# RioWong/PointCloudProcess

Measured on AMD Instinct MI355X. Metric: Mcorrespondences/s + ICP iter/s, 50M-vs-50M fp32 @ 1/2/4/8 MI355X, higher is better.
Workload: dtype f32

## Files before the change

include/pcp.h:

```cpp
#ifndef PCP_H
#define PCP_H

#include <stddef.h>
#include <stdint.h>

#ifdef __cplusplus
extern "C" {
#endif

#define PCP_ABI_VERSION 1

enum pcp_status {
    PCP_OK = 0,
    PCP_ERR_ARG = -1,
    PCP_ERR_HIP = -2,
    PCP_ERR_NOMEM = -3,
    PCP_ERR_EMPTY = -4,
    PCP_ERR_UNSUPPORTED = -5,
    PCP_ERR_ICP = -6,
    PCP_ERR_CAPACITY = -7
};

#define PCP_AOS48_STRIDE 48

// ... 139 lines not shown
                             int64_t nq, const uint64_t* keys_dev, const uint8_t* owner_dev, int rank,
                             int64_t lo, int64_t hi, const float* shard_xyz_dev, size_t shard_stride_bytes,
                             double* acc_dev);
int pcp_slab_guard(pcp_ctx* ctx, const double* T_dev, const double box_host[6], double lo,
                   double hi, int* flag_dev);
int pcp_icp_solve(const double acc_host[24], int do_scale, double dT_host[16]);
int pcp_icp_run(pcp_ctx* ctx, pcp_icp* icp, double T_inout[16], float rmax, int iters,
                int do_scale, double eps, float* err);
int pcp_icp_last_kernel_ms(const pcp_icp* icp, double* ms, int* launches);
int pcp_icp_step_dev(pcp_ctx* ctx, pcp_icp* icp, const double* T_dev, float rmax, double* acc_dev);
int pcp_icp_solve_dev(pcp_ctx* ctx, const double* acc_dev, int do_scale, double* T_dev, double* stats_dev);
int pcp_icp_run_dev(pcp_ctx* ctx, pcp_icp* icp, double* T_dev, float rmax, int iters, int do_scale,
                    double* stats_dev);
int pcp_icp_kernel_ms(pcp_ctx* ctx, pcp_icp* icp, double* ms, int* launches);
int pcp_icp_last_fallback(const pcp_icp* icp, int64_t* n);
int pcp_icp_last_searched(const pcp_icp* icp, int64_t* n);

int pcp_get_rot_icp(pcp_ctx* ctx, const void* src_aos48_dev, int64_t ns, int src_is_dense,
                    const void* temp_aos48_dev, int64_t nt, int temp_is_dense,
                    double mat_rot_host[16], float rmax, int iters, int do_scale,
                    double cell_size, float* err);

int pcp_pose_interpolate(double* rots_host, int64_t n, int64_t start, int64_t end);
int pcp_pose_lum_elch(double* rots_host, int64_t n, int64_t start, int64_t end, const double loop_host[16]);
int pcp_pose_loop_closure(double* ori_host, const uint64_t* ori_stamps_host, int64_t n_ori, const double* opt_host,
                          const uint64_t* opt_stamps_host, int64_t n_opt, int64_t window);

typedef struct pcp_grid pcp_grid;
int pcp_grid_create(pcp_ctx* ctx, pcp_grid** out);
int pcp_grid_destroy(pcp_grid* grid);
// ... 22 lines not shown
```

pointcloudprocess_amd/_lib.py:

```python
import ctypes as C
import os

HERE = os.path.dirname(os.path.abspath(__file__))
_AB = os.environ.get("PCP_AB") == "1" and bool(os.environ.get("PCP_LIB"))
LIB_PATH = os.environ["PCP_LIB"] if _AB else os.path.join(HERE, "libpcp.so")

PCP_OK = 0
_STATUS = {
    -1: "PCP_ERR_ARG", -2: "PCP_ERR_HIP", -3: "PCP_ERR_NOMEM", -4: "PCP_ERR_EMPTY",
    -5: "PCP_ERR_UNSUPPORTED", -6: "PCP_ERR_ICP", -7: "PCP_ERR_CAPACITY",
}

_vp, _i32, _i64, _sz, _f32, _f64, _u32 = (C.c_void_p, C.c_int, C.c_int64, C.c_size_t,
                                          C.c_float, C.c_double, C.c_uint32)
_P = C.POINTER
SIGNATURES = [
    ("pcp_abi_version", _i32, []),
    ("pcp_ctx_create", _i32, [_i32, _vp, _P(_vp)]),
    ("pcp_ctx_destroy", _i32, [_vp]),
    ("pcp_ctx_set_stream", _i32, [_vp, _vp]),
    ("pcp_ctx_stream", _vp, [_vp]),
    ("pcp_last_error", C.c_char_p, [_vp]),
    ("pcp_sync", _i32, [_vp]),
    ("pcp_malloc", _i32, [_vp, _P(_vp), _sz]),
# ... 57 lines not shown
    ("pcp_icp_keys", _i32, [_vp, _vp, _P(_f64), _f32, _i64, _vp]),
    ("pcp_icp_accumulate_keys", _i32, [_vp, _vp, _P(_f64), _vp, _i64, _i64, _vp, _sz, _vp]),
    ("pcp_icp_keys_dev", _i32, [_vp, _vp, _vp, _f32, _i64, _vp]),
    ("pcp_keys_owner", _i32, [_vp, _vp, _i64, _vp, _i32, _vp]),
    ("pcp_icp_accumulate_owned", _i32, [_vp, _vp, _vp, _sz, _i64, _vp, _vp, _i32, _i64, _i64, _vp, _sz, _vp]),
    ("pcp_slab_guard", _i32, [_vp, _vp, _P(_f64), _f64, _f64, _vp]),
    ("pcp_icp_solve", _i32, [_P(_f64), _i32, _P(_f64)]),
    ("pcp_icp_run", _i32, [_vp, _vp, _P(_f64), _f32, _i32, _i32, _f64, _P(_f32)]),
    ("pcp_icp_last_kernel_ms", _i32, [_vp, _P(_f64), _P(_i32)]),
    ("pcp_icp_step_dev", _i32, [_vp, _vp, _vp, _f32, _vp]),
    ("pcp_icp_solve_dev", _i32, [_vp, _vp, _i32, _vp, _vp]),
    ("pcp_icp_run_dev", _i32, [_vp, _vp, _vp, _f32, _i32, _i32, _vp]),
    ("pcp_icp_kernel_ms", _i32, [_vp, _vp, _P(_f64), _P(_i32)]),
    ("pcp_icp_last_fallback", _i32, [_vp, _P(_i64)]),
    ("pcp_icp_last_searched", _i32, [_vp, _P(_i64)]),
    ("pcp_fault_report_install", _i32, []),
    ("pcp_build_id", C.c_char_p, []),
    ("pcp_get_rot_icp", _i32, [_vp, _vp, _i64, _i32, _vp, _i64, _i32, _P(_f64), _f32, _i32, _i32,
                               _f64, _P(_f32)]),
]

_lib = None


class PcpError(RuntimeError):
    def __init__(self, code, msg):
        super().__init__(f"{_STATUS.get(code, code)}: {msg}")
        self.code = code


# ... 40 lines not shown
```

pointcloudprocess_amd/csrc/grid.hip:

```cpp
#include <cmath>
#include <vector>

#include <rocprim/device/device_radix_sort.hpp>
#include "sortcfg.hpp"

#include "grid.hpp"

namespace pcp {
namespace {

constexpr int kB = 256;

template <typename T>
__device__ __forceinline__ const T* pt_ptr(const T* base, size_t stride_bytes, int64_t i) {
    return (const T*)((const char*)base + (size_t)i * stride_bytes);
}

template <typename T>
__global__ void k_valid(const T* xyz, size_t stride, int64_t n_in, const int32_t* indices,
                        uint32_t* flag) {
    for (int64_t i = blockIdx.x * (int64_t)blockDim.x + threadIdx.x; i < n_in;
         i += (int64_t)gridDim.x * blockDim.x) {
        int64_t ci = indices ? indices[i] : i;
        const T* p = pt_ptr(xyz, stride, ci);
// ... 144 lines not shown
        bool on = (bits[i >> 5] >> (i & 31)) & 1u;
        brick[i] = on ? brick[i] : -1;
    }
}

constexpr int kChunk = 4096;
#ifndef PCP_SCAN_BLOCKS
#define PCP_SCAN_BLOCKS 16384
#endif
#ifndef PCP_BBOX_BLOCKS
#define PCP_BBOX_BLOCKS 4096
#endif
constexpr int64_t kScanBlocks = PCP_SCAN_BLOCKS;
constexpr int64_t kBboxBlocks = PCP_BBOX_BLOCKS;

__global__ void k_chunk_lo(const uint32_t* key, int64_t n, int64_t nchunk, uint32_t* lo) {
    for (int64_t p = blockIdx.x * (int64_t)blockDim.x + threadIdx.x; p <= n; p += (int64_t)gridDim.x * blockDim.x) {
        const int64_t kc = p < n ? (int64_t)key[p] : nchunk * kChunk;
        const int64_t kp = p > 0 ? (int64_t)key[p - 1] : -1;
        if (kc == kp) continue;
        const int64_t b0 = kp < 0 ? 0 : kp / kChunk + 1;
        const int64_t b1 = min(kc / kChunk, nchunk);
        for (int64_t b = b0; b <= b1; b++) lo[b] = (uint32_t)p;
    }
}

__global__ void __launch_bounds__(256) k_cell_starts(const uint32_t* __restrict__ key, const uint32_t* __restrict__ lo,
                                                     int64_t ncells1, uint32_t* __restrict__ cstart) {
    constexpr int kPer = kChunk / 256;
    __shared__ uint32_t s[kChunk];
    __shared__ uint32_t s_wmin[4];
    const int64_t c0 = (int64_t)blockIdx.x * kChunk;
// ... 38 lines not shown
        const int64_t c = c0 + e;
        if (c + 3 < ncells1) {
            *(uint4*)&cstart[c] = o;
        } else {
            if (c < ncells1) cstart[c] = o.x;
            if (c + 1 < ncells1) cstart[c + 1] = o.y;
            if (c + 2 < ncells1) cstart[c + 2] = o.z;
        }
    }
}

__global__ void k_far_sentinel(float4* pts, int64_t n) {
    pts[n] = make_float4(INFINITY, INFINITY, INFINITY, __int_as_float(0x7fffffff));
}

__global__ void k_cell_keys_rec(GridDesc g, const float* cxyz, size_t stride_f, const int32_t* mapping, int64_t n,
                                uint32_t* key, float4* rec, int32_t* mark) {
    for (int64_t i = blockIdx.x * (int64_t)blockDim.x + threadIdx.x; i < n;
         i += (int64_t)gridDim.x * blockDim.x) {
        const float* p = cxyz + stride_f * i;
        int cx, cy, cz;
        cell_of_point<float>(g, p, cx, cy, cz);
        key[i] = (uint32_t)cell_id(g, cx, cy, cz);
        rec[i] = make_float4(p[0], p[1], p[2], __int_as_float(mapping ? mapping[i] : (int32_t)i));
        if (mark) mark[brick_of(g, cx, cy, cz)] = 1;
    }
}


template <typename T>
__global__ void k_cell_keys(GridDesc g, const T* cxyz, size_t stride_t, int64_t n, uint32_t* key, uint32_t* val,
                            int32_t* mark) {
    for (int64_t i = blockIdx.x * (int64_t)blockDim.x + threadIdx.x; i < n;
         i += (int64_t)gridDim.x * blockDim.x) {
        int cx, cy, cz;
        cell_of_point<T>(g, cxyz + stride_t * i, cx, cy, cz);
        key[i] = (uint32_t)cell_id(g, cx, cy, cz);
        val[i] = (uint32_t)i;
        if (mark) mark[brick_of(g, cx, cy, cz)] = 1;
    }
}

// ... 169 lines not shown
    const int64_t dense_cap = std::min<int64_t>(((int64_t)1 << 31) - 2, std::max<int64_t>((int64_t)1 << 26, 16 * n));
    double ext[3];
    for (int a = 0; a < 3; a++) ext[a] = std::max(mx[a] - mn[a], 1e-9);
    const bool auto_h = !(cell_size > 0);
    double h = cell_size;
    if (auto_h) {
        const double target = 4.0;
        h = std::cbrt(ext[0] * ext[1] * ext[2] * target / std::max<double>((double)n, 1.0));
        double emax = std::max(ext[0], std::max(ext[1], ext[2]));
        if (!(h > emax * 1e-7)) h = emax * 1e-7;
        if (!(h > 0)) h = 1.0;
    }
    uint32_t* count = nullptr;
    uint32_t* rank = nullptr;
    uint32_t* skey = nullptr;
    if ((is_f64 && (rc = dmalloc(ctx, &rank, n + 1))) || (rc = dmalloc(ctx, &skey, n + 1))) {
        dfree(ctx, rank);
        dfree(ctx, cxyz);
        return fail(rc);
    }
    if ((rc = dmalloc(ctx, (typename Real<T>::V4**)&ix->pts, n + 1))) {
        dfree(ctx, rank); dfree(ctx, skey); dfree(ctx, cxyz);
        return fail(rc);
    }
    bool hooked = false;
    for (int attempt = 0; attempt < 3; attempt++) {
        GridDesc g{};
        while (!make_geometry(g, mn, mx, h, cap)) h *= 2.0;
        dfree(ctx, ix->brick); ix->brick = nullptr;
        dfree(ctx, count); count = nullptr;
        const int64_t ncells_dense = (int64_t)g.n[0] * g.n[1] * g.n[2];
// ... 46 lines not shown
            if (occ > 12.0) { h *= std::sqrt(4.0 / occ); redo = true; }
            else if (occ < 1.5) { h *= std::cbrt(4.0 / occ); redo = true; }
            if (redo) continue;
        }
        if (on_geom && *on_geom && !hooked) {
            hooked = true;
            if ((rc = (*on_geom)(g))) break;
        }
        if ((rc = dmalloc(ctx, &count, ncells + 2))) break;
        uint32_t* key1 = nullptr;
        uint32_t* val1 = nullptr;
        using V4 = typename Real<T>::V4;
        if (n > 0) {
            if ((rc = dmalloc(ctx, &key1, n))) break;
            if (is_f64 && (rc = dmalloc(ctx, &val1, n))) { dfree(ctx, key1); break; }
            float4* rec0 = nullptr;
            if (!is_f64 && (rc = dmalloc(ctx, &rec0, n))) { dfree(ctx, key1); break; }
            unsigned bits = 1;
            while (bits < 32 && ((uint64_t)1 << bits) <= (uint64_t)ncells) bits++;
            size_t tmp_bytes = 0;
            void* tmp = nullptr;
            if (is_f64) {
                hipLaunchKernelGGL(k_cell_keys<T>, dim3(grid_for(n, kB)), dim3(kB), 0, st, g, direct ? xyz : cxyz,
                                   direct ? stride / sizeof(T) : (size_t)3, n, skey, rank, g.dense ? ix->brick : nullptr);
                PCP_HIP(ctx, rocprim::radix_sort_pairs(nullptr, tmp_bytes, skey, key1, rank, val1, (size_t)n, 0u,
                                                       bits, st));
                if (!(rc = dmalloc(ctx, (char**)&tmp, tmp_bytes)))
                    PCP_HIP(ctx, rocprim::radix_sort_pairs(tmp, tmp_bytes, skey, key1, rank, val1, (size_t)n, 0u,
                                                           bits, st));
            } else {
                if (direct)
                    hipLaunchKernelGGL(k_cell_keys_rec, dim3(grid_for(n, kB)), dim3(kB), 0, st, g, (const float*)xyz,
                                       stride / sizeof(float), (const int32_t*)nullptr, n, skey, rec0, nullptr);
                else
                    hipLaunchKernelGGL(k_cell_keys_rec, dim3(grid_for(n, kB)), dim3(kB), 0, st, g, (const float*)cxyz,
                                       (size_t)3, (const int32_t*)ix->mapping, n, skey, rec0, nullptr);
                PCP_HIP(ctx, rocprim::radix_sort_pairs<RecSortConfig>(nullptr, tmp_bytes, skey, key1, rec0, (float4*)ix->pts,
                                                       (size_t)n, 0u, bits, st));
                if (!(rc = dmalloc(ctx, (char**)&tmp, tmp_bytes)))
                    PCP_HIP(ctx, rocprim::radix_sort_pairs<RecSortConfig>(tmp, tmp_bytes, skey, key1, rec0, (float4*)ix->pts,
                                                           (size_t)n, 0u, bits, st));
            }
            dfree(ctx, tmp);
            dfree(ctx, rec0);
            if (rc) { dfree(ctx, key1); dfree(ctx, val1); break; }
            if (!is_f64)
                hipLaunchKernelGGL(k_far_sentinel, dim3(1), dim3(1), 0, st, (float4*)ix->pts, n);
        }
        if (g.dense && is_f64)
            hipLaunchKernelGGL(k_brick_flag, dim3(grid_for(g.nbricks, kB)), dim3(kB), 0, st, ix->brick, g.nbricks);
        const int64_t nchunk = (ncells + 1 + kChunk - 1) / kChunk;
        uint32_t* lo = nullptr;
        if ((rc = dmalloc(ctx, &lo, nchunk + 1))) {
            dfree(ctx, key1); dfree(ctx, val1);
            break;
        }
        hipLaunchKernelGGL(k_chunk_lo, dim3(grid_for(n + 1, kB, kScanBlocks)), dim3(kB), 0, st, (const uint32_t*)key1, n,
                           nchunk, lo);
        hipLaunchKernelGGL(k_cell_starts, dim3((unsigned)nchunk), dim3(kB), 0, st, (const uint32_t*)key1,
                           (const uint32_t*)lo, ncells + 1, count);
        dfree(ctx, lo);
        g.cstart = count;
        if (g.dense && is_f64 && n > 0)
            hipLaunchKernelGGL(k_brick_rows, dim3(grid_for(g.nbricks, kB)), dim3(kB), 0, st, g, ix->brick);
        ix->g = g;
        ix->cstart = count;
        count = nullptr;
        if (is_f64) {
            if ((rc = dmalloc(ctx, &ix->sorted_j, n + 1))) { dfree(ctx, key1); dfree(ctx, val1); break; }
            if (n > 0)
                hipLaunchKernelGGL(k_gather<T>, dim3(grid_for(n, kB)), dim3(kB), 0, st, direct ? xyz : cxyz,
                                   direct ? stride / sizeof(T) : (size_t)3, (const uint32_t*)val1,
                                   (const int32_t*)ix->mapping, n, (V4*)ix->pts, ix->sorted_j, is_f64);
// ... 72 lines not shown
```

pointcloudprocess_amd/csrc/icp.hip:

```cpp
#include <cmath>
#include <cstdlib>
#include <cstring>
#include <vector>

#include <rocprim/device/device_radix_sort.hpp>
#include <rocprim/device/device_select.hpp>
#include <rocprim/iterator/counting_iterator.hpp>
#include "sortcfg.hpp"

#include "grid.hpp"
#include "wave_acc.hpp"

namespace pcp {
struct QXyz {
    float x, y, z;
};
}

struct pcp_icp {
    pcp_ctx* ctx = nullptr;
    pcp_ctx* owner = nullptr;
    const pcp_index* target = nullptr;
    int64_t nq = 0;
    int64_t nq_in = 0;
    pcp::QXyz* q = nullptr;
    int32_t* qidx = nullptr;
    uint32_t* cand = nullptr;
    bool narrow = false;
    float* pose_hist = nullptr;
    int64_t launches = 0;
    bool last_verified = false;
    int32_t* sv = nullptr;
    uint32_t* sv_count = nullptr;
    uint32_t* sv_off = nullptr;
    int32_t* svc = nullptr;
    int64_t sv_seg = 0;
    int64_t nseg_v = 0;
    int nb_ver = 0;
    int32_t* fb = nullptr;
    uint32_t* fb_count = nullptr;
    uint32_t* fb_off = nullptr;
// ... 1383 lines not shown
    if (!(mn >= lo && mx <= hi)) *flag = 1;
}

#ifndef PCP_QKEY_LOCAL
#define PCP_QKEY_LOCAL 1
#endif
#ifndef PCP_QBRICK
#define PCP_QBRICK 8
#endif
__host__ __device__ inline int64_t qbricks(const GridDesc& g, int a) { return (g.n[a] + PCP_QBRICK - 1) / PCP_QBRICK; }
__host__ __device__ inline uint32_t query_key_end(const GridDesc& g) {
    if (PCP_QBRICK != 4)
        return (uint32_t)(qbricks(g, 0) * qbricks(g, 1) * qbricks(g, 2) * PCP_QBRICK * PCP_QBRICK * PCP_QBRICK);
    return (uint32_t)(PCP_QKEY_LOCAL ? g.nbricks * 64 : g.nbricks);
}
__global__ void k_query_keys(GridDesc g, const float* q, size_t stride_f, int64_t n, uint32_t* key, float4* rec) {
    for (int64_t i = blockIdx.x * (int64_t)blockDim.x + threadIdx.x; i < n; i += (int64_t)gridDim.x * blockDim.x) {
        const float* p = q + (size_t)i * stride_f;
        const float x = p[0], y = p[1], z = p[2];
        const bool fin = isfinite(x) && isfinite(y) && isfinite(z);
        uint32_t k = query_key_end(g);
        if (fin) {
            const int cx = clampi((int)floorf(cell_f<float>(g, x, 0) - 0.5f), 0, g.n[0] - 1);
            const int cy = clampi((int)floorf(cell_f<float>(g, y, 1) - 0.5f), 0, g.n[1] - 1);
            const int cz = clampi((int)floorf(cell_f<float>(g, z, 2) - 0.5f), 0, g.n[2] - 1);
            if (PCP_QBRICK != 4) {
                constexpr int B = PCP_QBRICK;
                const int64_t b = ((int64_t)(cz / B) * qbricks(g, 1) + cy / B) * qbricks(g, 0) + cx / B;
                k = (uint32_t)(b * B * B * B + ((cz % B) * B + cy % B) * B + cx % B);
            } else {
                k = PCP_QKEY_LOCAL ? (uint32_t)(brick_of(g, cx, cy, cz) * 64 + local_of(cx, cy, cz))
                                   : (uint32_t)brick_of(g, cx, cy, cz);
            }
        }
        key[i] = k;
        rec[i] = make_float4(x, y, z, __int_as_float((int)i));
    }
}

__global__ void k_split_queries(const float4* qs, int64_t n, QXyz* q, int32_t* qi) {
    for (int64_t i = blockIdx.x * (int64_t)blockDim.x + threadIdx.x; i < n; i += (int64_t)gridDim.x * blockDim.x) {
        const float4 v = qs[i];
        q[i] = QXyz{v.x, v.y, v.z};
        qi[i] = __float_as_int(v.w);
    }
}

__global__ void k_first_at_least(const uint32_t* sorted, int64_t n, uint32_t key, unsigned long long* out) {
    int64_t lo = 0, hi = n;
    while (lo < hi) {
        const int64_t mid = (lo + hi) >> 1;
        if (sorted[mid] < key) lo = mid + 1;
        else hi = mid;
    }
    *out = (unsigned long long)lo;
}

__host__ __device__ void svd3(const double Ain[9], double U[9], double s[3], double V[9]) {
    double A[9];
    for (int i = 0; i < 9; i++) A[i] = Ain[i];
    for (int i = 0; i < 9; i++) V[i] = (i % 4 == 0) ? 1.0 : 0.0;
// ... 326 lines not shown

int pcp_icp_check_sizes(int64_t n_target, int64_t nq) {
    if (n_target < 0 || nq < 0) return PCP_ERR_ARG;
    if (nq >= ((int64_t)1 << 31)) return PCP_ERR_ARG;
    if (n_target + 1 >= ((int64_t)1 << 28)) return PCP_ERR_CAPACITY;
    return PCP_OK;
}

}

namespace pcp {
namespace {

struct QuerySort {
    uint32_t *k0 = nullptr, *k1 = nullptr;
    float4 *r0 = nullptr, *qs = nullptr;
    unsigned long long* d_cnt = nullptr;
    void* tmp = nullptr;
    hipEvent_t done = nullptr;
    int64_t nq = 0;
    void release(pcp_ctx* ctx) {
        dfree(ctx, k0); dfree(ctx, k1); dfree(ctx, r0); dfree(ctx, qs); dfree(ctx, d_cnt); dfree(ctx, tmp);
        k0 = k1 = nullptr; r0 = qs = nullptr; d_cnt = nullptr; tmp = nullptr;
        if (done) event_put(ctx, done);
        done = nullptr;
    }
};

int icp_check_grid(pcp_ctx* ctx, const GridDesc& g, int64_t n_target, int64_t nq) {
    if (int rc = pcp_icp_check_sizes(n_target, nq))
        return set_error(ctx, rc, rc == PCP_ERR_CAPACITY ? "ICP target must have < 2^28 - 1 points (32-bit record offsets)"
                                                         : "ICP supports < 2^31 queries");
    if (g.nbricks * 64 >= ((int64_t)1 << 32) ||
        qbricks(g, 0) * qbricks(g, 1) * qbricks(g, 2) * PCP_QBRICK * PCP_QBRICK * PCP_QBRICK >= ((int64_t)1 << 32))
        return set_error(ctx, PCP_ERR_UNSUPPORTED, "ICP target grid too large for 32-bit cell keys");
    return PCP_OK;
}

int qsort_launch(pcp_ctx* ctx, hipStream_t st, const GridDesc& g, const float* q, size_t q_stride, int64_t nq,
                 QuerySort& s) {
    s.nq = nq;
    int rc = PCP_OK;
    if ((rc = dmalloc(ctx, &s.k0, nq)) || (rc = dmalloc(ctx, &s.k1, nq)) || (rc = dmalloc(ctx, &s.r0, nq)) ||
        (rc = dmalloc(ctx, &s.qs, nq + 1)) || (rc = dmalloc(ctx, &s.d_cnt, 1)))
        return rc;
    PCP_HIP(ctx, event_get(ctx, &s.done));
    unsigned bits = 1;
    while (bits < 32 && ((uint64_t)1 << bits) <= (uint64_t)query_key_end(g)) bits++;
    size_t tb = 0;
    if (nq > 0) {
        PCP_HIP(ctx, rocprim::radix_sort_pairs<RecSortConfig>(nullptr, tb, s.k0, s.k1, s.r0, s.qs, (size_t)nq, 0u, bits, st));
        if ((rc = dmalloc(ctx, (char**)&s.tmp, tb))) return rc;
    }
    if (st != ctx->stream) {
        hipEvent_t go = nullptr;
        PCP_HIP(ctx, event_get(ctx, &go));
        hipError_t e = hipEventRecord(go, ctx->stream);
        if (e == hipSuccess) e = hipStreamWaitEvent(st, go, 0);
        event_put(ctx, go);
        if (e != hipSuccess) return hip_fail(ctx, e, "query sort stream order", __FILE__, __LINE__);
    }
    PCP_HIP(ctx, hipMemsetAsync(s.d_cnt, 0, sizeof(unsigned long long), st));
    if (nq > 0) {
        hipLaunchKernelGGL(k_query_keys, dim3(grid_for(nq, 256)), dim3(256), 0, st, g, q, q_stride / sizeof(float), nq,
                           s.k0, s.r0);
        PCP_HIP(ctx, rocprim::radix_sort_pairs<RecSortConfig>(s.tmp, tb, s.k0, s.k1, s.r0, s.qs, (size_t)nq, 0u, bits, st));
        hipLaunchKernelGGL(k_first_at_least, dim3(1), dim3(1), 0, st, s.k1, nq, query_key_end(g), s.d_cnt);
    }
    PCP_HIP(ctx, hipGetLastError());
    PCP_HIP(ctx, hipEventRecord(s.done, st));
    return PCP_OK;
}

int qsort_finish(pcp_ctx* ctx, QuerySort& s, QXyz** q3, int32_t** qi, int64_t* nfin) {
    PCP_HIP(ctx, hipStreamWaitEvent(ctx->stream, s.done, 0));
    unsigned long long hc = 0;
    PCP_HIP(ctx, hipMemcpyAsync(&hc, s.d_cnt, sizeof(hc), hipMemcpyDeviceToHost, ctx->stream));
    PCP_HIP(ctx, hipStreamSynchronize(ctx->stream));
    *nfin = (int64_t)hc;
    int rc = PCP_OK;
    if ((rc = dmalloc(ctx, q3, s.nq + 1)) || (rc = dmalloc(ctx, qi, s.nq + 1))) return rc;
    if (*nfin > 0)
        hipLaunchKernelGGL(k_split_queries, dim3(grid_for(*nfin, 256)), dim3(256), 0, ctx->stream,
                           (const float4*)s.qs, *nfin, *q3, *qi);
    PCP_HIP(ctx, hipGetLastError());
    return PCP_OK;
}

int icp_make(pcp_ctx* ctx, const pcp_index* target, QXyz* q3, int32_t* qi, int64_t nfin, int64_t nq, pcp_icp** out) {
    pcp_icp* icp = new pcp_icp();
    icp->ctx = ctx;
    icp->owner = ctx;
    ctx_retain(ctx);
    icp->target = target;
    icp->nq = nfin;
    icp->nq_in = nq;
    icp->q = q3;
    icp->qidx = qi;
    int dev_cus = 256;
    int cus = 0;
    if (hipDeviceGetAttribute(&cus, hipDeviceAttributeMultiprocessorCount, ctx->device) == hipSuccess && cus > 0)
        dev_cus = cus;
    const int64_t want = (icp->nq + kIcpBlock - 1) / kIcpBlock;
    icp->nb_fast = (int)std::max<int64_t>(1, std::min<int64_t>(want, (int64_t)dev_cus * PCP_OCT_WAVES));
    icp->nb_fast_l = (int)std::max<int64_t>(1, std::min<int64_t>(icp->nb_fast, (int64_t)dev_cus * PCP_OCT_WAVES_LIST));
    icp->nb_ring = (int)std::max<int64_t>(1, std::min<int64_t>(want, (int64_t)dev_cus * PCP_RING_WAVES));
    const int64_t nwaves = (int64_t)icp->nb_fast * (kIcpBlock / 64);
    const int64_t nwaves_l = (int64_t)icp->nb_fast_l * (kIcpBlock / 64);
    const int64_t nchunks64 = (icp->nq + 63) / 64;
    icp->fb_seg = ((nchunks64 + nwaves_l - 1) / nwaves_l) * 64;
    icp->nb_ver = (int)std::max<int64_t>(1, std::min<int64_t>(want, (int64_t)dev_cus * PCP_VER_WAVES));
    const int64_t nwaves_v = (int64_t)icp->nb_ver * (kIcpBlock / 64);
    icp->sv_seg = ((nchunks64 + nwaves_v - 1) / nwaves_v) * 64;
// ... 40 lines not shown
}

extern "C" {

int pcp_icp_create(pcp_ctx* ctx, const pcp_index* target, const float* q, size_t q_stride, int64_t nq,
                   pcp_icp** out) {
    if (!ctx || !target || !out || nq < 0 || (nq > 0 && !q)) return PCP_ERR_ARG;
    if (target->is_f64) return pcp::set_error(ctx, PCP_ERR_ARG, "ICP target must be an fp32 index");
    PCP_HIP(ctx, hipSetDevice(ctx->device));
    *out = nullptr;
    if (q_stride == 0) q_stride = 3 * sizeof(float);
    if (q_stride % sizeof(float)) return pcp::set_error(ctx, PCP_ERR_ARG, "query stride must be whole floats");
    PCP_TRY(pcp::icp_check_grid(ctx, target->g, target->n, nq));
    pcp::QuerySort s;
    pcp::QXyz* q3 = nullptr;
    int32_t* qi = nullptr;
    int64_t nfin = 0;
    int rc = pcp::qsort_launch(ctx, ctx->stream, target->g, q, q_stride, nq, s);
    if (!rc) rc = pcp::qsort_finish(ctx, s, &q3, &qi, &nfin);
    s.release(ctx);
    if (rc) {
        pcp::dfree(ctx, q3);
        pcp::dfree(ctx, qi);
        return rc;
    }
    return pcp::icp_make(ctx, target, q3, qi, nfin, nq, out);
}

int pcp_icp_create_with_target(pcp_ctx* ctx, const float* target_xyz, size_t t_stride, int64_t n_target,
                               double cell_size, const float* q, size_t q_stride, int64_t nq, pcp_index** index_out,
                               pcp_icp** icp_out) {
    if (!ctx || !index_out || !icp_out || nq < 0 || (nq > 0 && !q) || n_target < 0 || (n_target > 0 && !target_xyz))
        return PCP_ERR_ARG;
    PCP_HIP(ctx, hipSetDevice(ctx->device));
    *index_out = nullptr;
    *icp_out = nullptr;
    if (q_stride == 0) q_stride = 3 * sizeof(float);
    if (q_stride % sizeof(float)) return pcp::set_error(ctx, PCP_ERR_ARG, "query stride must be whole floats");
    pcp::QuerySort s;
    bool launched = false;
    const pcp::GeomHook hook = [&](const pcp::GridDesc& g) -> int {
        PCP_TRY(pcp::icp_check_grid(ctx, g, n_target, nq));
        hipStream_t side = nullptr;
        PCP_TRY(pcp::side_stream(ctx, &side));
        launched = true;
        return pcp::qsort_launch(ctx, side, g, q, q_stride, nq, s);
    };
    pcp_index* ix = nullptr;
    int rc = pcp::index_build_f32_hooked(ctx, target_xyz, t_stride, n_target, cell_size, &ix, hook);
    pcp::QXyz* q3 = nullptr;
    int32_t* qi = nullptr;
    int64_t nfin = 0;
    if (!rc && !launched) rc = pcp::qsort_launch(ctx, ctx->stream, ix->g, q, q_stride, nq, s);
    if (!rc) rc = pcp::qsort_finish(ctx, s, &q3, &qi, &nfin);
    if (rc && launched) (void)hipStreamSynchronize(ctx->side);
    s.release(ctx);
    if (!rc) rc = pcp::icp_make(ctx, ix, q3, qi, nfin, nq, icp_out);
    else {
        pcp::dfree(ctx, q3);
        pcp::dfree(ctx, qi);
    }
    if (rc) {
        if (ix) pcp_index_destroy(ix);
        return rc;
    }
    *index_out = ix;
    return PCP_OK;
}

int pcp_icp_set_options(pcp_icp* icp, int oct_lanes_first, int oct_lanes_list, int ring_lanes, int ablate) {
    if (!icp) return PCP_ERR_ARG;
    auto lanes = [](int v) { return v == 0 || v == 1 || v == 2 || v == 4 || v == 8; };
    pcp_ctx* ctx = icp->owner;
    if (!lanes(oct_lanes_first) || !lanes(oct_lanes_list) || !lanes(ring_lanes) || ablate < 0)
        return pcp::set_error(ctx, PCP_ERR_ARG, "pcp_icp_set_options: lanes must be 0, 1, 2, 4 or 8; ablate >= 0");
    const bool widen = (ablate & PCP_ICP_OPT_WIDE_CACHE) && icp->narrow;
// ... 20 lines not shown
    icp->ring_g = ring_lanes;
    icp->dbg = ablate & ~(PCP_ICP_OPT_WIDE_CACHE | PCP_ICP_OPT_GRAPH);
    icp->graph = (ablate & PCP_ICP_OPT_GRAPH) != 0;
    return PCP_OK;
}

int pcp_icp_destroy(pcp_icp* icp) {
    if (!icp) return PCP_ERR_ARG;
    (void)hipSetDevice(icp->owner->device);
    if (icp->gexec) {
        (void)hipStreamSynchronize(icp->ctx->stream);
        (void)hipGraphExecDestroy(icp->gexec);
    }
    pcp::dfree(icp->owner, icp->q);
    pcp::dfree(icp->owner, icp->qidx);
    pcp::dfree(icp->owner, icp->partials);
    pcp::dfree(icp->owner, icp->acc);
    pcp::dfree(icp->owner, icp->cand);
    pcp::dfree(icp->owner, icp->pose_hist);
    pcp::dfree(icp->owner, icp->sv);
    pcp::dfree(icp->owner, icp->sv_count);
    pcp::dfree(icp->owner, icp->sv_off);
    pcp::dfree(icp->owner, icp->svc);

    pcp::dfree(icp->owner, icp->fb);
    pcp::dfree(icp->owner, icp->fb_count);
    pcp::dfree(icp->owner, icp->fb_off);
    pcp::dfree(icp->owner, icp->fbc);
    pcp::dfree(icp->owner, icp->pose_dev);
    pcp::event_put(icp->owner, icp->ev0);
// ... 3 lines not shown
    for (auto& pr : icp->tev) {
        pcp::event_put(icp->owner, pr.first);
        pcp::event_put(icp->owner, pr.second);
    }
    pcp_ctx* owner = icp->owner;
    delete icp;
    pcp::ctx_release(owner);
    return PCP_OK;
}

int pcp_icp_step(pcp_ctx* ctx, pcp_icp* icp, const double T[16], float rmax, double* acc_dev,
                 int32_t* corr_idx, float* corr_d2) {
    if (!ctx || !icp || !T || !acc_dev || (corr_idx && !corr_d2) || !(rmax >= 0.f)) return PCP_ERR_ARG;
    PCP_HIP(ctx, hipSetDevice(ctx->device));
    icp->ctx = ctx;
    PCP_TRY(pcp::icp_launch(icp, T, rmax, acc_dev, corr_idx, corr_d2));
    double fbn = 0.0;
    PCP_HIP(ctx, hipMemcpyAsync(&fbn, acc_dev + 23, sizeof(double), hipMemcpyDeviceToHost, ctx->stream));
    uint32_t nsv = (uint32_t)icp->nq;
    if (icp->last_verified)
        PCP_HIP(ctx, hipMemcpyAsync(&nsv, icp->sv_off + icp->nseg_v, sizeof(nsv),
                                    hipMemcpyDeviceToHost, ctx->stream));
    PCP_HIP(ctx, hipStreamSynchronize(ctx->stream));
    icp->last_fallback = (uint32_t)fbn;
    icp->last_searched = nsv;
    float ms = 0.f;
    PCP_HIP(ctx, hipEventElapsedTime(&ms, icp->ev0, icp->ev1));
    icp->last_ms = ms;
    icp->last_launches = 1;
    if (icp->dbg) {
// ... 1 lines not shown
        (void)hipEventElapsedTime(&m1, icp->ev0, icp->ev_mid);
        (void)hipEventElapsedTime(&mv, icp->ev0, icp->ev_ver);
        std::fprintf(stderr, "[pcp icp dbg=%d] verify %.4f ms  octant %.4f ms  fallback %.4f ms  searched %u  "
                     "n_fallback %u\n", icp->dbg, mv, m1 - mv, ms - m1, nsv, icp->last_fallback);
    }
    return PCP_OK;
}

int pcp_icp_keys(pcp_ctx* ctx, pcp_icp* icp, const double T[16], float rmax, int64_t target_offset,
                 uint64_t* keys_dev) {
    if (!ctx || !icp || !T || !keys_dev || !(rmax >= 0.f) || target_offset < 0 ||
        target_offset + pcp_index_size(icp->target) > ((int64_t)1 << 32))
        return PCP_ERR_ARG;
    PCP_HIP(ctx, hipSetDevice(ctx->device));
    icp->ctx = ctx;
    const int saved = icp->dbg;
    icp->dbg |= pcp::kDbgNoAccum;
    pcp::IcpArgs a{};
    const int rc = pcp::icp_launch(icp, T, rmax, icp->acc, nullptr, nullptr, nullptr, &a);
    icp->dbg = saved;
    PCP_TRY(rc);
    if (icp->nq_in > icp->nq)
        hipLaunchKernelGGL(pcp::k_fill_keys, dim3(pcp::grid_for(icp->nq_in, 256)), dim3(256), 0, ctx->stream, keys_dev,
                           icp->nq_in);
    if (icp->nq > 0)
        hipLaunchKernelGGL(pcp::k_make_keys, dim3(pcp::grid_for(icp->nq, 256)), dim3(256), 0, ctx->stream, a,
                           (uint32_t)target_offset, keys_dev);
    PCP_LAUNCH_CHECK(ctx);
    return PCP_OK;
}

int pcp_icp_keys_dev(pcp_ctx* ctx, pcp_icp* icp, const double* T_dev, float rmax, int64_t target_offset,
                     uint64_t* keys_dev) {
    if (!ctx || !icp || !T_dev || !keys_dev || !(rmax >= 0.f) || target_offset < 0 ||
        target_offset + pcp_index_size(icp->target) > ((int64_t)1 << 32))
        return PCP_ERR_ARG;
    PCP_HIP(ctx, hipSetDevice(ctx->device));
    icp->ctx = ctx;
    const int saved = icp->dbg;
    icp->dbg |= pcp::kDbgNoAccum;
    pcp::IcpArgs a{};
    const int rc = pcp::icp_launch(icp, nullptr, rmax, icp->acc, nullptr, nullptr, T_dev, &a);
    icp->dbg = saved;
    PCP_TRY(rc);
    if (icp->nq_in > icp->nq)
        hipLaunchKernelGGL(pcp::k_fill_keys, dim3(pcp::grid_for(icp->nq_in, 256)), dim3(256), 0, ctx->stream, keys_dev,
                           icp->nq_in);
    if (icp->nq > 0)
        hipLaunchKernelGGL(pcp::k_make_keys, dim3(pcp::grid_for(icp->nq, 256)), dim3(256), 0, ctx->stream, a,
                           (uint32_t)target_offset, keys_dev);
    PCP_LAUNCH_CHECK(ctx);
    return PCP_OK;
}
// ... 37 lines not shown
    PCP_HIP(ctx, hipSetDevice(ctx->device));
    hipLaunchKernelGGL(pcp::k_slab_guard, dim3(1), dim3(1), 0, ctx->stream, T_dev, box[0], box[1], box[2], box[3],
                       box[4], box[5], lo, hi, flag_dev);
    PCP_LAUNCH_CHECK(ctx);
    return PCP_OK;
}

int pcp_icp_accumulate_keys(pcp_ctx* ctx, pcp_icp* icp, const double T[16], const uint64_t* keys_dev,
                            int64_t lo, int64_t hi, const float* shard_xyz_dev, size_t shard_stride_bytes,
                            double* acc_dev) {
    if (!ctx || !icp || !T || !keys_dev || !acc_dev || lo < 0 || hi < lo || (hi > lo && !shard_xyz_dev))
        return PCP_ERR_ARG;
    if (shard_stride_bytes == 0) shard_stride_bytes = 3 * sizeof(float);
    if (shard_stride_bytes % sizeof(float)) return pcp::set_error(ctx, PCP_ERR_ARG, "shard stride must be whole floats");
    PCP_HIP(ctx, hipSetDevice(ctx->device));
    pcp::IcpArgs a{};
    for (int r = 0; r < 3; r++) {
        for (int c = 0; c < 3; c++) a.R[3 * r + c] = (float)T[4 * r + c];
        a.t[r] = (float)T[4 * r + 3];
    }
    const int nb = (int)std::min<int64_t>(std::max<int64_t>(1, (icp->nq + 255) / 256), icp->nb_fast + icp->nb_ring);
    hipLaunchKernelGGL(pcp::k_acc_keys, dim3(nb), dim3(256), 0, ctx->stream, icp->q, icp->qidx, icp->nq, keys_dev,
                       (uint64_t)lo, (uint64_t)hi, shard_xyz_dev, shard_stride_bytes / sizeof(float), a,
                       icp->partials);
    hipLaunchKernelGGL(pcp::k_sum_partials, dim3(1), dim3(256), 0, ctx->stream, (const double*)icp->partials, nb,
                       acc_dev);
    PCP_LAUNCH_CHECK(ctx);
    return PCP_OK;
}

// ... 90 lines not shown
    return PCP_OK;
}

int pcp_icp_last_fallback(const pcp_icp* icp, int64_t* n) {
    if (!icp || !n) return PCP_ERR_ARG;
    *n = icp->last_fallback;
    return PCP_OK;
}

int pcp_icp_last_searched(const pcp_icp* icp, int64_t* n) {
    if (!icp || !n) return PCP_ERR_ARG;
    *n = icp->last_searched;
    return PCP_OK;
}

int pcp_icp_last_kernel_ms(const pcp_icp* icp, double* ms, int* launches) {
    if (!icp) return PCP_ERR_ARG;
    if (ms) *ms = icp->last_ms;
    if (launches) *launches = icp->last_launches;
    return PCP_OK;
}

}
```

pointcloudprocess_amd/ops.py:

```python
import ctypes as C

import numpy as np
import torch

from . import _lib
from ._lib import check

POINT48 = np.dtype(
    [("x", "<f8"), ("y", "<f8"), ("z", "<f8"), ("w", "<f8"), ("rgba", "<u4"),
     ("stamp_id", "<u4"), ("pad", "<u4", (2,))])
PLANE = np.dtype([("normal_x", "<f4"), ("normal_y", "<f4"), ("normal_z", "<f4"),
                  ("min_value", "<f4"), ("curvature", "<f4"), ("distance", "<f4")])


def _ptr(t):
    return C.c_void_p(t.data_ptr()) if t is not None else None


class Context:

    def __init__(self, device=0):
        self.lib = _lib.load()
        self.device = torch.device("cuda", device) if isinstance(device, int) else torch.device(device)
        idx = self.device.index or 0
# ... 372 lines not shown
    def last_kernel_ms(self):
        ms, n = C.c_double(), C.c_int()
        self.ctx.check(self.ctx.lib.pcp_icp_last_kernel_ms(self.h, C.byref(ms), C.byref(n)))
        return ms.value, n.value

    def last_searched(self):
        n = C.c_int64()
        self.ctx.check(self.ctx.lib.pcp_icp_last_searched(self.h, C.byref(n)))
        return n.value

    def last_fallback(self):
        n = C.c_int64()
        self.ctx.check(self.ctx.lib.pcp_icp_last_fallback(self.h, C.byref(n)))
        return n.value

    def close(self):
        if getattr(self, "h", None):
            self.ctx.lib.pcp_icp_destroy(self.h)
            self.h = None

    def __del__(self):
        self.close()


def keys_owner(ctx, keys, bounds, out=None):
    n = keys.numel()
    out = torch.empty(n, dtype=torch.uint8, device=ctx.device) if out is None else out
    assert keys.dtype == torch.int64 and bounds.dtype == torch.int64 and out.numel() >= n
    ctx.check(ctx.lib.pcp_keys_owner(ctx.h, _ptr(keys), n, _ptr(bounds), bounds.numel() - 1, _ptr(out)))
    return out
# ... 34 lines not shown
```

Baseline: 28540.

## Sort raw query xyz directly and defer query index permutation until needed

Query and target sorting now feed rocprim radix sort through transform iterators that compute keys and records on the fly, which removes the staging float4 record buffers and the split kernel. The sorted query payload shrinks to 12-byte xyz, and the original-index permutation is rebuilt lazily by a second key sort only when correspondence indices or sharded accumulation need it. The aim is to cut memory traffic and allocations during ICP setup. Paths that need indices now pay an extra sort on first use, and a sorted_queries API is added.

```diff
diff --git a/include/pcp.h b/include/pcp.h
--- a/include/pcp.h
+++ b/include/pcp.h
@@ -177,6 +177,8 @@
                     double* stats_dev);
 int pcp_icp_kernel_ms(pcp_ctx* ctx, pcp_icp* icp, double* ms, int* launches);
 int pcp_icp_last_fallback(const pcp_icp* icp, int64_t* n);
+int pcp_icp_sorted_queries(pcp_ctx* ctx, pcp_icp* icp, float* xyz_out_dev, int32_t* idx_out_dev,
+                           int64_t* n_finite);
 int pcp_icp_last_searched(const pcp_icp* icp, int64_t* n);
 
 int pcp_get_rot_icp(pcp_ctx* ctx, const void* src_aos48_dev, int64_t ns, int src_is_dense,
diff --git a/pointcloudprocess_amd/_lib.py b/pointcloudprocess_amd/_lib.py
--- a/pointcloudprocess_amd/_lib.py
+++ b/pointcloudprocess_amd/_lib.py
@@ -95,6 +95,7 @@
     ("pcp_icp_kernel_ms", _i32, [_vp, _vp, _P(_f64), _P(_i32)]),
     ("pcp_icp_last_fallback", _i32, [_vp, _P(_i64)]),
     ("pcp_icp_last_searched", _i32, [_vp, _P(_i64)]),
+    ("pcp_icp_sorted_queries", _i32, [_vp, _vp, _vp, _vp, _P(_i64)]),
     ("pcp_fault_report_install", _i32, []),
     ("pcp_build_id", C.c_char_p, []),
     ("pcp_get_rot_icp", _i32, [_vp, _vp, _i64, _i32, _vp, _i64, _i32, _P(_f64), _f32, _i32, _i32,
diff --git a/pointcloudprocess_amd/csrc/grid.hip b/pointcloudprocess_amd/csrc/grid.hip
--- a/pointcloudprocess_amd/csrc/grid.hip
+++ b/pointcloudprocess_amd/csrc/grid.hip
@@ -1,7 +1,10 @@
 #include <cmath>
+#include <cstring>
 #include <vector>
 
 #include <rocprim/device/device_radix_sort.hpp>
+#include <rocprim/iterator/counting_iterator.hpp>
+#include <rocprim/iterator/transform_iterator.hpp>
 #include "sortcfg.hpp"
 
 #include "grid.hpp"
@@ -182,8 +185,9 @@
 constexpr int64_t kScanBlocks = PCP_SCAN_BLOCKS;
 constexpr int64_t kBboxBlocks = PCP_BBOX_BLOCKS;
 
-__global__ void k_chunk_lo(const uint32_t* key, int64_t n, int64_t nchunk, uint32_t* lo) {
+__global__ void k_chunk_lo(const uint32_t* key, int64_t n, int64_t nchunk, uint32_t* lo, uint32_t* pad) {
     for (int64_t p = blockIdx.x * (int64_t)blockDim.x + threadIdx.x; p <= n; p += (int64_t)gridDim.x * blockDim.x) {
+        if (p == n) *pad = (uint32_t)n;
         const int64_t kc = p < n ? (int64_t)key[p] : nchunk * kChunk;
         const int64_t kp = p > 0 ? (int64_t)key[p - 1] : -1;
         if (kc == kp) continue;
@@ -252,18 +256,27 @@
     pts[n] = make_float4(INFINITY, INFINITY, INFINITY, __int_as_float(0x7fffffff));
 }
 
-__global__ void k_cell_keys_rec(GridDesc g, const float* cxyz, size_t stride_f, const int32_t* mapping, int64_t n,
-                                uint32_t* key, float4* rec, int32_t* mark) {
-    for (int64_t i = blockIdx.x * (int64_t)blockDim.x + threadIdx.x; i < n;
-         i += (int64_t)gridDim.x * blockDim.x) {
-        const float* p = cxyz + stride_f * i;
+struct CellKeyOf {
+    GridDesc g;
+    const float* xyz;
+    size_t stride_f;
+    __device__ __forceinline__ uint32_t operator()(int64_t i) const {
         int cx, cy, cz;
-        cell_of_point<float>(g, p, cx, cy, cz);
-        key[i] = (uint32_t)cell_id(g, cx, cy, cz);
-        rec[i] = make_float4(p[0], p[1], p[2], __int_as_float(mapping ? mapping[i] : (int32_t)i));
-        if (mark) mark[brick_of(g, cx, cy, cz)] = 1;
-    }
-}
+        cell_of_point<float>(g, xyz + stride_f * i, cx, cy, cz);
+        return (uint32_t)cell_id(g, cx, cy, cz);
+    }
+};
+struct CellRecOf {
+    const float* xyz;
+    size_t stride_f;
+    const int32_t* mapping;
+    __device__ __forceinline__ float4 operator()(int64_t i) const {
+        const float* p = xyz + stride_f * i;
+        return make_float4(p[0], p[1], p[2], __int_as_float(mapping ? mapping[i] : (int32_t)i));
+    }
+};
+using CellKeyIt = rocprim::transform_iterator<rocprim::counting_iterator<int64_t>, CellKeyOf, uint32_t>;
+using CellRecIt = rocprim::transform_iterator<rocprim::counting_iterator<int64_t>, CellRecOf, float4>;
 
 
 template <typename T>
@@ -463,7 +476,7 @@
     uint32_t* count = nullptr;
     uint32_t* rank = nullptr;
     uint32_t* skey = nullptr;
-    if ((is_f64 && (rc = dmalloc(ctx, &rank, n + 1))) || (rc = dmalloc(ctx, &skey, n + 1))) {
+    if (is_f64 && ((rc = dmalloc(ctx, &rank, n + 1)) || (rc = dmalloc(ctx, &skey, n + 1)))) {
         dfree(ctx, rank);
         dfree(ctx, cxyz);
         return fail(rc);
@@ -540,8 +553,6 @@
         if (n > 0) {
             if ((rc = dmalloc(ctx, &key1, n))) break;
             if (is_f64 && (rc = dmalloc(ctx, &val1, n))) { dfree(ctx, key1); break; }
-            float4* rec0 = nullptr;
-            if (!is_f64 && (rc = dmalloc(ctx, &rec0, n))) { dfree(ctx, key1); break; }
             unsigned bits = 1;
             while (bits < 32 && ((uint64_t)1 << bits) <= (uint64_t)ncells) bits++;
             size_t tmp_bytes = 0;
@@ -555,20 +566,18 @@
                     PCP_HIP(ctx, rocprim::radix_sort_pairs(tmp, tmp_bytes, skey, key1, rank, val1, (size_t)n, 0u,
                                                            bits, st));
             } else {
-                if (direct)
-                    hipLaunchKernelGGL(k_cell_keys_rec, dim3(grid_for(n, kB)), dim3(kB), 0, st, g, (const float*)xyz,
-                                       stride / sizeof(float), (const int32_t*)nullptr, n, skey, rec0, nullptr);
-                else
-                    hipLaunchKernelGGL(k_cell_keys_rec, dim3(grid_for(n, kB)), dim3(kB), 0, st, g, (const float*)cxyz,
-                                       (size_t)3, (const int32_t*)ix->mapping, n, skey, rec0, nullptr);
-                PCP_HIP(ctx, rocprim::radix_sort_pairs<RecSortConfig>(nullptr, tmp_bytes, skey, key1, rec0, (float4*)ix->pts,
-                                                       (size_t)n, 0u, bits, st));
+                const float* src = direct ? (const float*)xyz : (const float*)cxyz;
+                const size_t src_stride = direct ? stride / sizeof(float) : (size_t)3;
+                const rocprim::counting_iterator<int64_t> first(0);
+                const CellKeyIt keys_in(first, CellKeyOf{g, src, src_stride});
+                const CellRecIt recs_in(first, CellRecOf{src, src_stride, direct ? nullptr : (const int32_t*)ix->mapping});
+                PCP_HIP(ctx, rocprim::radix_sort_pairs<RecSortConfig>(nullptr, tmp_bytes, keys_in, key1, recs_in,
+                                                                      (float4*)ix->pts, (size_t)n, 0u, bits, st));
                 if (!(rc = dmalloc(ctx, (char**)&tmp, tmp_bytes)))
-                    PCP_HIP(ctx, rocprim::radix_sort_pairs<RecSortConfig>(tmp, tmp_bytes, skey, key1, rec0, (float4*)ix->pts,
-                                                           (size_t)n, 0u, bits, st));
+                    PCP_HIP(ctx, rocprim::radix_sort_pairs<RecSortConfig>(tmp, tmp_bytes, keys_in, key1, recs_in,
+                                                                          (float4*)ix->pts, (size_t)n, 0u, bits, st));
             }
             dfree(ctx, tmp);
-            dfree(ctx, rec0);
             if (rc) { dfree(ctx, key1); dfree(ctx, val1); break; }
             if (!is_f64)
                 hipLaunchKernelGGL(k_far_sentinel, dim3(1), dim3(1), 0, st, (float4*)ix->pts, n);
@@ -582,7 +591,7 @@
             break;
         }
         hipLaunchKernelGGL(k_chunk_lo, dim3(grid_for(n + 1, kB, kScanBlocks)), dim3(kB), 0, st, (const uint32_t*)key1, n,
-                           nchunk, lo);
+                           nchunk, lo, count + ncells + 1);
         hipLaunchKernelGGL(k_cell_starts, dim3((unsigned)nchunk), dim3(kB), 0, st, (const uint32_t*)key1,
                            (const uint32_t*)lo, ncells + 1, count);
         dfree(ctx, lo);
diff --git a/pointcloudprocess_amd/csrc/icp.hip b/pointcloudprocess_amd/csrc/icp.hip
--- a/pointcloudprocess_amd/csrc/icp.hip
+++ b/pointcloudprocess_amd/csrc/icp.hip
@@ -6,6 +6,7 @@
 #include <rocprim/device/device_radix_sort.hpp>
 #include <rocprim/device/device_select.hpp>
 #include <rocprim/iterator/counting_iterator.hpp>
+#include <rocprim/iterator/transform_iterator.hpp>
 #include "sortcfg.hpp"
 
 #include "grid.hpp"
@@ -25,6 +26,8 @@
     int64_t nq_in = 0;
     pcp::QXyz* q = nullptr;
     int32_t* qidx = nullptr;
+    uint32_t* qkey = nullptr;
+    unsigned qbits = 0;
     uint32_t* cand = nullptr;
     bool narrow = false;
     float* pose_hist = nullptr;
@@ -1438,7 +1441,7 @@
         return (uint32_t)(qbricks(g, 0) * qbricks(g, 1) * qbricks(g, 2) * PCP_QBRICK * PCP_QBRICK * PCP_QBRICK);
     return (uint32_t)(PCP_QKEY_LOCAL ? g.nbricks * 64 : g.nbricks);
 }
-__global__ void k_query_keys(GridDesc g, const float* q, size_t stride_f, int64_t n, uint32_t* key, float4* rec) {
+__global__ void k_query_keys(GridDesc g, const float* q, size_t stride_f, int64_t n, uint32_t* key) {
     for (int64_t i = blockIdx.x * (int64_t)blockDim.x + threadIdx.x; i < n; i += (int64_t)gridDim.x * blockDim.x) {
         const float* p = q + (size_t)i * stride_f;
         const float x = p[0], y = p[1], z = p[2];
@@ -1458,17 +1461,18 @@
             }
         }
         key[i] = k;
-        rec[i] = make_float4(x, y, z, __int_as_float((int)i));
-    }
-}
-
-__global__ void k_split_queries(const float4* qs, int64_t n, QXyz* q, int32_t* qi) {
-    for (int64_t i = blockIdx.x * (int64_t)blockDim.x + threadIdx.x; i < n; i += (int64_t)gridDim.x * blockDim.x) {
-        const float4 v = qs[i];
-        q[i] = QXyz{v.x, v.y, v.z};
-        qi[i] = __float_as_int(v.w);
-    }
-}
+    }
+}
+
+struct QXyzAt {
+    const float* q;
+    size_t stride_f;
+    __device__ __forceinline__ QXyz operator()(int64_t i) const {
+        const float* p = q + (size_t)i * stride_f;
+        return QXyz{p[0], p[1], p[2]};
+    }
+};
+using QXyzIt = rocprim::transform_iterator<rocprim::counting_iterator<int64_t>, QXyzAt, QXyz>;
 
 __global__ void k_first_at_least(const uint32_t* sorted, int64_t n, uint32_t key, unsigned long long* out) {
     int64_t lo = 0, hi = n;
@@ -1825,18 +1829,27 @@
 
 struct QuerySort {
     uint32_t *k0 = nullptr, *k1 = nullptr;
-    float4 *r0 = nullptr, *qs = nullptr;
+    QXyz* q = nullptr;
     unsigned long long* d_cnt = nullptr;
     void* tmp = nullptr;
     hipEvent_t done = nullptr;
     int64_t nq = 0;
+    unsigned bits = 0;
     void release(pcp_ctx* ctx) {
-        dfree(ctx, k0); dfree(ctx, k1); dfree(ctx, r0); dfree(ctx, qs); dfree(ctx, d_cnt); dfree(ctx, tmp);
-        k0 = k1 = nullptr; r0 = qs = nullptr; d_cnt = nullptr; tmp = nullptr;
+        dfree(ctx, k0); dfree(ctx, k1); dfree(ctx, q); dfree(ctx, d_cnt); dfree(ctx, tmp);
+        k0 = k1 = nullptr; q = nullptr; d_cnt = nullptr; tmp = nullptr;
         if (done) event_put(ctx, done);
         done = nullptr;
     }
 };
+
+hipError_t qsort_pairs(void* tmp, size_t& tb, const float* q, size_t q_stride, QuerySort& s, hipStream_t st) {
+    if (q_stride == sizeof(QXyz))
+        return rocprim::radix_sort_pairs<RecSortConfig>(tmp, tb, s.k0, s.k1, (const QXyz*)q, s.q, (size_t)s.nq, 0u,
+                                                        s.bits, st);
+    const QXyzIt vals(rocprim::counting_iterator<int64_t>(0), QXyzAt{q, q_stride / sizeof(float)});
+    return rocprim::radix_sort_pairs<RecSortConfig>(tmp, tb, s.k0, s.k1, vals, s.q, (size_t)s.nq, 0u, s.bits, st);
+}
 
 int icp_check_grid(pcp_ctx* ctx, const GridDesc& g, int64_t n_target, int64_t nq) {
     if (int rc = pcp_icp_check_sizes(n_target, nq))
@@ -1852,15 +1865,15 @@
                  QuerySort& s) {
     s.nq = nq;
     int rc = PCP_OK;
-    if ((rc = dmalloc(ctx, &s.k0, nq)) || (rc = dmalloc(ctx, &s.k1, nq)) || (rc = dmalloc(ctx, &s.r0, nq)) ||
-        (rc = dmalloc(ctx, &s.qs, nq + 1)) || (rc = dmalloc(ctx, &s.d_cnt, 1)))
+    if ((rc = dmalloc(ctx, &s.k0, nq)) || (rc = dmalloc(ctx, &s.k1, nq)) || (rc = dmalloc(ctx, &s.q, nq + 1)) ||
+        (rc = dmalloc(ctx, &s.d_cnt, 1)))
         return rc;
     PCP_HIP(ctx, event_get(ctx, &s.done));
-    unsigned bits = 1;
-    while (bits < 32 && ((uint64_t)1 << bits) <= (uint64_t)query_key_end(g)) bits++;
+    s.bits = 1;
+    while (s.bits < 32 && ((uint64_t)1 << s.bits) <= (uint64_t)query_key_end(g)) s.bits++;
     size_t tb = 0;
     if (nq > 0) {
-        PCP_HIP(ctx, rocprim::radix_sort_pairs<RecSortConfig>(nullptr, tb, s.k0, s.k1, s.r0, s.qs, (size_t)nq, 0u, bits, st));
+        PCP_HIP(ctx, qsort_pairs(nullptr, tb, q, q_stride, s, st));
         if ((rc = dmalloc(ctx, (char**)&s.tmp, tb))) return rc;
     }
     if (st != ctx->stream) {
@@ -1874,8 +1887,8 @@
     PCP_HIP(ctx, hipMemsetAsync(s.d_cnt, 0, sizeof(unsigned long long), st));
     if (nq > 0) {
         hipLaunchKernelGGL(k_query_keys, dim3(grid_for(nq, 256)), dim3(256), 0, st, g, q, q_stride / sizeof(float), nq,
-                           s.k0, s.r0);
-        PCP_HIP(ctx, rocprim::radix_sort_pairs<RecSortConfig>(s.tmp, tb, s.k0, s.k1, s.r0, s.qs, (size_t)nq, 0u, bits, st));
+                           s.k0);
+        PCP_HIP(ctx, qsort_pairs(s.tmp, tb, q, q_stride, s, st));
         hipLaunchKernelGGL(k_first_at_least, dim3(1), dim3(1), 0, st, s.k1, nq, query_key_end(g), s.d_cnt);
     }
     PCP_HIP(ctx, hipGetLastError());
@@ -1883,22 +1896,52 @@
     return PCP_OK;
 }
 
-int qsort_finish(pcp_ctx* ctx, QuerySort& s, QXyz** q3, int32_t** qi, int64_t* nfin) {
+int qsort_finish(pcp_ctx* ctx, QuerySort& s, QXyz** q3, uint32_t** qk, int64_t* nfin) {
     PCP_HIP(ctx, hipStreamWaitEvent(ctx->stream, s.done, 0));
     unsigned long long hc = 0;
     PCP_HIP(ctx, hipMemcpyAsync(&hc, s.d_cnt, sizeof(hc), hipMemcpyDeviceToHost, ctx->stream));
     PCP_HIP(ctx, hipStreamSynchronize(ctx->stream));
     *nfin = (int64_t)hc;
-    int rc = PCP_OK;
-    if ((rc = dmalloc(ctx, q3, s.nq + 1)) || (rc = dmalloc(ctx, qi, s.nq + 1))) return rc;
-    if (*nfin > 0)
-        hipLaunchKernelGGL(k_split_queries, dim3(grid_for(*nfin, 256)), dim3(256), 0, ctx->stream,
-                           (const float4*)s.qs, *nfin, *q3, *qi);
-    PCP_HIP(ctx, hipGetLastError());
+    *q3 = s.q;
+    *qk = s.k0;
+    s.q = nullptr;
+    s.k0 = nullptr;
     return PCP_OK;
 }
 
-int icp_make(pcp_ctx* ctx, const pcp_index* target, QXyz* q3, int32_t* qi, int64_t nfin, int64_t nq, pcp_icp** out) {
+int icp_need_qidx(pcp_ctx* ctx, pcp_icp* icp) {
+    if (icp->qidx) return PCP_OK;
+    pcp_ctx* owner = icp->owner;
+    if (ctx != owner) PCP_HIP(ctx, hipStreamSynchronize(owner->stream));
+    const int64_t n = icp->nq_in;
+    int32_t* idx = nullptr;
+    uint32_t* ksorted = nullptr;
+    void* tmp = nullptr;
+    int rc = dmalloc(owner, &idx, n + 1);
+    if (!rc && n > 0) {
+        size_t tb = 0;
+        const rocprim::counting_iterator<int32_t> pos(0);
+        hipError_t e = rocprim::radix_sort_pairs(nullptr, tb, icp->qkey, ksorted, pos, idx, (size_t)n, 0u, icp->qbits,
+                                                 ctx->stream);
+        if (e == hipSuccess && !(rc = dmalloc(owner, &ksorted, n)) && !(rc = dmalloc(owner, (char**)&tmp, tb)))
+            e = rocprim::radix_sort_pairs(tmp, tb, icp->qkey, ksorted, pos, idx, (size_t)n, 0u, icp->qbits, ctx->stream);
+        if (e == hipSuccess && !rc && ctx != owner) e = hipStreamSynchronize(ctx->stream);
+        if (e != hipSuccess) rc = hip_fail(ctx, e, "query index sort", __FILE__, __LINE__);
+    }
+    dfree(owner, tmp);
+    dfree(owner, ksorted);
+    if (rc) {
+        dfree(owner, idx);
+        return rc;
+    }
+    dfree(owner, icp->qkey);
+    icp->qkey = nullptr;
+    icp->qidx = idx;
+    return PCP_OK;
+}
+
+int icp_make(pcp_ctx* ctx, const pcp_index* target, QXyz* q3, uint32_t* qk, unsigned qbits, int64_t nfin, int64_t nq,
+             pcp_icp** out) {
     pcp_icp* icp = new pcp_icp();
     icp->ctx = ctx;
     icp->owner = ctx;
@@ -1907,7 +1950,8 @@
     icp->nq = nfin;
     icp->nq_in = nq;
     icp->q = q3;
-    icp->qidx = qi;
+    icp->qkey = qk;
+    icp->qbits = qbits;
     int dev_cus = 256;
     int cus = 0;
     if (hipDeviceGetAttribute(&cus, hipDeviceAttributeMultiprocessorCount, ctx->device) == hipSuccess && cus > 0)
@@ -1978,17 +2022,13 @@
     PCP_TRY(pcp::icp_check_grid(ctx, target->g, target->n, nq));
     pcp::QuerySort s;
     pcp::QXyz* q3 = nullptr;
-    int32_t* qi = nullptr;
+    uint32_t* qk = nullptr;
     int64_t nfin = 0;
     int rc = pcp::qsort_launch(ctx, ctx->stream, target->g, q, q_stride, nq, s);
-    if (!rc) rc = pcp::qsort_finish(ctx, s, &q3, &qi, &nfin);
+    if (!rc) rc = pcp::qsort_finish(ctx, s, &q3, &qk, &nfin);
     s.release(ctx);
-    if (rc) {
-        pcp::dfree(ctx, q3);
-        pcp::dfree(ctx, qi);
-        return rc;
-    }
-    return pcp::icp_make(ctx, target, q3, qi, nfin, nq, out);
+    if (rc) return rc;
+    return pcp::icp_make(ctx, target, q3, qk, s.bits, nfin, nq, out);
 }
 
 int pcp_icp_create_with_target(pcp_ctx* ctx, const float* target_xyz, size_t t_stride, int64_t n_target,
@@ -2013,17 +2053,13 @@
     pcp_index* ix = nullptr;
     int rc = pcp::index_build_f32_hooked(ctx, target_xyz, t_stride, n_target, cell_size, &ix, hook);
     pcp::QXyz* q3 = nullptr;
-    int32_t* qi = nullptr;
+    uint32_t* qk = nullptr;
     int64_t nfin = 0;
     if (!rc && !launched) rc = pcp::qsort_launch(ctx, ctx->stream, ix->g, q, q_stride, nq, s);
-    if (!rc) rc = pcp::qsort_finish(ctx, s, &q3, &qi, &nfin);
+    if (!rc) rc = pcp::qsort_finish(ctx, s, &q3, &qk, &nfin);
     if (rc && launched) (void)hipStreamSynchronize(ctx->side);
     s.release(ctx);
-    if (!rc) rc = pcp::icp_make(ctx, ix, q3, qi, nfin, nq, icp_out);
-    else {
-        pcp::dfree(ctx, q3);
-        pcp::dfree(ctx, qi);
-    }
+    if (!rc) rc = pcp::icp_make(ctx, ix, q3, qk, s.bits, nfin, nq, icp_out);
     if (rc) {
         if (ix) pcp_index_destroy(ix);
         return rc;
@@ -2074,6 +2110,7 @@
     }
     pcp::dfree(icp->owner, icp->q);
     pcp::dfree(icp->owner, icp->qidx);
+    pcp::dfree(icp->owner, icp->qkey);
     pcp::dfree(icp->owner, icp->partials);
     pcp::dfree(icp->owner, icp->acc);
     pcp::dfree(icp->owner, icp->cand);
@@ -2107,6 +2144,7 @@
     if (!ctx || !icp || !T || !acc_dev || (corr_idx && !corr_d2) || !(rmax >= 0.f)) return PCP_ERR_ARG;
     PCP_HIP(ctx, hipSetDevice(ctx->device));
     icp->ctx = ctx;
+    if (corr_idx) PCP_TRY(pcp::icp_need_qidx(ctx, icp));
     PCP_TRY(pcp::icp_launch(icp, T, rmax, acc_dev, corr_idx, corr_d2));
     double fbn = 0.0;
     PCP_HIP(ctx, hipMemcpyAsync(&fbn, acc_dev + 23, sizeof(double), hipMemcpyDeviceToHost, ctx->stream));
@@ -2138,6 +2176,7 @@
         return PCP_ERR_ARG;
     PCP_HIP(ctx, hipSetDevice(ctx->device));
     icp->ctx = ctx;
+    PCP_TRY(pcp::icp_need_qidx(ctx, icp));
     const int saved = icp->dbg;
     icp->dbg |= pcp::kDbgNoAccum;
     pcp::IcpArgs a{};
@@ -2161,6 +2200,7 @@
         return PCP_ERR_ARG;
     PCP_HIP(ctx, hipSetDevice(ctx->device));
     icp->ctx = ctx;
+    PCP_TRY(pcp::icp_need_qidx(ctx, icp));
     const int saved = icp->dbg;
     icp->dbg |= pcp::kDbgNoAccum;
     pcp::IcpArgs a{};
@@ -2228,6 +2268,7 @@
     if (shard_stride_bytes == 0) shard_stride_bytes = 3 * sizeof(float);
     if (shard_stride_bytes % sizeof(float)) return pcp::set_error(ctx, PCP_ERR_ARG, "shard stride must be whole floats");
     PCP_HIP(ctx, hipSetDevice(ctx->device));
+    PCP_TRY(pcp::icp_need_qidx(ctx, icp));
     pcp::IcpArgs a{};
     for (int r = 0; r < 3; r++) {
         for (int c = 0; c < 3; c++) a.R[3 * r + c] = (float)T[4 * r + c];
@@ -2348,6 +2389,20 @@
     return PCP_OK;
 }
 
+int pcp_icp_sorted_queries(pcp_ctx* ctx, pcp_icp* icp, float* xyz_out_dev, int32_t* idx_out_dev, int64_t* n_finite) {
+    if (!ctx || !icp) return PCP_ERR_ARG;
+    PCP_HIP(ctx, hipSetDevice(ctx->device));
+    if (idx_out_dev) PCP_TRY(pcp::icp_need_qidx(ctx, icp));
+    if (xyz_out_dev && icp->nq > 0)
+        PCP_HIP(ctx, hipMemcpyAsync(xyz_out_dev, icp->q, (size_t)icp->nq * sizeof(pcp::QXyz), hipMemcpyDeviceToDevice,
+                                    ctx->stream));
+    if (idx_out_dev && icp->nq > 0)
+        PCP_HIP(ctx, hipMemcpyAsync(idx_out_dev, icp->qidx, (size_t)icp->nq * sizeof(int32_t), hipMemcpyDeviceToDevice,
+                                    ctx->stream));
+    if (n_finite) *n_finite = icp->nq;
+    return PCP_OK;
+}
+
 int pcp_icp_last_kernel_ms(const pcp_icp* icp, double* ms, int* launches) {
     if (!icp) return PCP_ERR_ARG;
     if (ms) *ms = icp->last_ms;
diff --git a/pointcloudprocess_amd/ops.py b/pointcloudprocess_amd/ops.py
--- a/pointcloudprocess_amd/ops.py
+++ b/pointcloudprocess_amd/ops.py
@@ -410,6 +410,14 @@
         self.ctx.check(self.ctx.lib.pcp_icp_last_fallback(self.h, C.byref(n)))
         return n.value
 
+    def sorted_queries(self):
+        ctx = self.ctx
+        xyz = torch.empty((self.nq_in, 3), dtype=torch.float32, device=ctx.device)
+        idx = torch.empty(self.nq_in, dtype=torch.int32, device=ctx.device)
+        n = C.c_int64()
+        ctx.check(ctx.lib.pcp_icp_sorted_queries(ctx.h, self.h, _ptr(xyz), _ptr(idx), C.byref(n)))
+        return xyz[:n.value], idx[:n.value]
+
     def close(self):
         if getattr(self, "h", None):
             self.ctx.lib.pcp_icp_destroy(self.h)
```

Result: no change. 28690, median of 6 (+0.5%).
